# AssemblyAI-Community/MinImagen

Measured on NVIDIA H100. Metric: denoising steps/sec (SR256 U-Net, batch 32 per GPU per step), higher is better.
Workload: dtype f16 tensor-core operands, f32 accumulate / residual stream

## Files before the change

### minimagen_b200/csrc/conv_tc.cu

```cuda
#include "conv_tc.cuh"

#include <cuda_runtime.h>
#include <mutex>
#include <stdio.h>

#include "kernels.cuh"
#include "launch.cuh"
#include "ptx.cuh"
#include "sat_half.cuh"
#include "wgmma.cuh"

namespace mi {

namespace {

constexpr int kNumThreads = 384;
constexpr uint32_t kABytes = kConvBlockM * kConvBlockK * 2;
constexpr uint32_t kRingBudget = 192 * 1024;
constexpr uint32_t kAuxBytes = 512;
constexpr uint32_t kSmemMax = 227 * 1024;
constexpr int kProducerRegs = 40;
constexpr int kConsumerRegs = 232;
static_assert(128 * kProducerRegs + 256 * kConsumerRegs <= 65536, "register file overcommitted");
constexpr int kTurnBar = 2;
constexpr int kStatBar = 4;
constexpr uint32_t stat_scratch_bytes(int block_n) { return 2 * 4 * (block_n / 16 > 0 ? block_n / 16 : 1) * 2 * 8; }

template <int BLOCK_N>
struct Cfg {
    static constexpr uint32_t kBBytes = BLOCK_N * kConvBlockK * 2;
    static constexpr uint32_t kStageBytes = kABytes + kBBytes;
    static constexpr int kStages = (kRingBudget / kStageBytes) > 8 ? 8 : (kRingBudget / kStageBytes);
    static constexpr uint32_t kSmemBytes = kStages * kStageBytes + 1024  + kAuxBytes;
};

__device__ __forceinline__ float silu(float v) { return __fdividef(v, 1.0f + __expf(-v)); }

template <int BLOCK_N, bool GN, bool TR = false>
__global__ void __launch_bounds__(kNumThreads, 1)
conv_wg_kernel(const __grid_constant__ CUtensorMap tmA, const __grid_constant__ CUtensorMap tmA2,
               const __grid_constant__ CUtensorMap tmB, const __grid_constant__ CUtensorMap tmX,
               const __grid_constant__ CUtensorMap tmX2, const __grid_constant__ ConvTcArgs args,
               const __grid_constant__ GnPrologueArgs gn) {
    using C = Cfg<BLOCK_N>;
    constexpr int STAGES = C::kStages;
    static_assert(2 * STAGES * 8 <= 256, "barrier block overlaps the GroupNorm scratch");
    static_assert(!TR || (BLOCK_N == 256 && !GN), "the transposed tile is the cooperative 256-wide one");
    constexpr bool PP = !GN && !TR && BLOCK_N <= 128;
    constexpr int HALVES = PP ? 2 : 1;
    constexpr int TILE_PIX = TR ? BLOCK_N : kConvBlockM;

    extern __shared__ uint8_t smem_raw[];
    uint8_t* smem = reinterpret_cast<uint8_t*>((reinterpret_cast<uintptr_t>(smem_raw) + 1023) & ~uintptr_t(1023));
    uint64_t* bars = reinterpret_cast<uint64_t*>(smem + STAGES * C::kStageBytes);
    uint64_t* full_bar = bars;
    uint64_t* empty_bar = bars + STAGES;

    const int warp = threadIdx.x >> 5;
    const int lane = threadIdx.x & 31;
    const int wg = threadIdx.x >> 7;
    int* err = args.err_flag;

    if (threadIdx.x == 0) {
        ptx::prefetch_tensormap(&tmB);
        if (!GN) {
            ptx::prefetch_tensormap(&tmA);
            ptx::prefetch_tensormap(&tmA2);
        }
        for (int i = 0; i < STAGES; ++i) {
            ptx::mbar_init(&full_bar[i], GN ? 5 : 1);
            ptx::mbar_init(&empty_bar[i], PP ? 1 : 2);
        }
        ptx::fence_barrier_init();
    }
    __syncthreads();
    pdl_wait();

    const int num_tap_kb = args.num_taps * args.chunks_per_tap;
    const int num_kb = num_tap_kb + args.x_chunks;
    const int tiles_m = args.tiles_w * args.tiles_h * args.tiles_b;
    const int total_tiles = tiles_m * args.tiles_n;
    const int BW = 1 << args.bw_log2, BH = 1 << args.bh_log2;
    const int BB = TILE_PIX >> (args.bw_log2 + args.bh_log2);

    if (wg == 0) {
        if constexpr (!GN) {
            ptx::setmaxnreg_dec<kProducerRegs>();
            if (warp == 0) {
                int stage = 0;
                uint32_t phase = 0;
                for (int tile = blockIdx.x; tile < total_tiles; tile += gridDim.x) {
                    const int nt = tile % args.tiles_n;
                    const int mt = tile / args.tiles_n;
                    const int w0 = (mt % args.tiles_w) * BW;
                    const int h0 = ((mt / args.tiles_w) % args.tiles_h) * BH;
                    const int b0 = (mt / (args.tiles_w * args.tiles_h)) * BB;
                    const int n0 = nt * BLOCK_N;
                    for (int kb = 0; kb < num_kb; ++kb) {
                        ptx::mbar_wait(&empty_bar[stage], phase ^ 1, err, 100 + stage);
                        if (ptx::elect_one()) {
                            uint8_t* sa = smem + stage * C::kStageBytes + (TR ? kABytes : 0);
                            uint8_t* sb = smem + stage * C::kStageBytes + (TR ? 0 : kABytes);
                            ptx::mbar_arrive_expect_tx(&full_bar[stage], C::kStageBytes);
                            if (kb < num_tap_kb) {
                                const int t = kb / args.chunks_per_tap, j = kb - t * args.chunks_per_tap;
                                const int cw = w0 * args.in_stride + args.dw[t], ch = h0 * args.in_stride + args.dh[t];
                                if (j < args.a_split)
                                    ptx::tma_load_5d(&tmA, &full_bar[stage], sa, args.a_chan_off + j * kConvBlockK, cw, ch,
                                                     args.ph[t], b0);
                                else
                                    ptx::tma_load_5d(&tmA2, &full_bar[stage], sa,
                                                     args.a_chan_off2 + (j - args.a_split) * kConvBlockK, cw, ch, args.ph[t], b0);
                            } else {
                                const int jx = kb - num_tap_kb;
                                if (jx < args.x_split)
                                    ptx::tma_load_5d(&tmX, &full_bar[stage], sa, args.x_chan_off + jx * kConvBlockK, w0, h0, 0, b0);
                                else
                                    ptx::tma_load_5d(&tmX2, &full_bar[stage], sa,
                                                     args.x_chan_off2 + (jx - args.x_split) * kConvBlockK, w0, h0, 0, b0);
                            }
                            ptx::tma_load_2d(&tmB, &full_bar[stage], sb, kb * kConvBlockK, n0);
                        }
                        if (++stage == STAGES) { stage = 0; phase ^= 1; }
                    }
                }
                pdl_trigger();
            }
        } else {
            float* s_mean = reinterpret_cast<float*>(reinterpret_cast<uint8_t*>(bars) + 256);
            float* s_rstd = s_mean + 32;
            float* sA = reinterpret_cast<float*>(reinterpret_cast<uint8_t*>(bars) + kAuxBytes);
            const int tt = threadIdx.x;
            const int lq = tt & 7;
            const int prow = tt >> 3;
            const int C0 = gn.C0, C1 = gn.C1, Ctot = C0 + C1, Cg = Ctot / gn.groups;
            const int H = args.H, W = args.W;
            float* sB = sA + Ctot;
            int stage = 0;
            uint32_t phase = 0;
            int cur_b = -1;
            for (int tile = blockIdx.x; tile < total_tiles; tile += gridDim.x) {
                const int nt = tile % args.tiles_n;
                const int mt = tile / args.tiles_n;
                const int w0 = (mt % args.tiles_w) * BW;
                const int h0 = ((mt / args.tiles_w) % args.tiles_h) * BH;
                const int b = mt / (args.tiles_w * args.tiles_h);
                const int n0 = nt * BLOCK_N;
                if (b != cur_b) {
                    ptx::bar_sync(1, 128);
                    if (tt < gn.groups) {
                        const int g = tt;
                        double su = 0.0, sq = 0.0;
                        const int lo = g * Cg, hi = lo + Cg;
                        const int lo0 = min(lo, C0), hi0 = min(hi, C0);
                        for (int e = lo0 / 16; e < hi0 / 16; ++e) {
                            su += gn.stats0[((long long)b * (C0 / 16) + e) * 2];
                            sq += gn.stats0[((long long)b * (C0 / 16) + e) * 2 + 1];
                        }
                        const int lo1 = max(lo, C0) - C0, hi1 = max(hi, C0) - C0;
                        for (int e = lo1 / 16; e < hi1 / 16; ++e) {
                            su += (double)gn.scale1 * gn.stats1[((long long)b * (C1 / 16) + e) * 2];
                            sq += (double)gn.scale1 * (double)gn.scale1 * gn.stats1[((long long)b * (C1 / 16) + e) * 2 + 1];
                        }
                        const double n = (double)Cg * H * W;
                        const double mean = su / n;
                        double var = sq / n - mean * mean;
                        if (var < 0) var = 0;
                        s_mean[g] = (float)mean;
                        s_rstd[g] = (float)(1.0 / sqrt(var + (double)gn.eps));
                    }
                    ptx::bar_sync(1, 128);
                    for (int cc = tt; cc < Ctot; cc += 128) {
                        const int g = cc / Cg;
                        float a = s_rstd[g] * gn.gamma[cc];
                        float bb = gn.beta[cc] - s_mean[g] * a;
                        if (gn.scale_shift) {
                            const float sc = gn.scale_shift[(long long)b * gn.ss_ld + cc] + 1.0f;
                            const float shv = gn.scale_shift[(long long)b * gn.ss_ld + Ctot + cc];
                            a *= sc;
                            bb = bb * sc + shv;
                        }
                        if (cc >= C0) a *= gn.scale1;
                        sA[cc] = a;
                        sB[cc] = bb;
                    }
                    cur_b = b;
                    ptx::bar_sync(1, 128);
                }
                const long long img = (long long)b * H * W;
                for (int kb = 0; kb < num_kb; ++kb) {
                    const int t = kb / args.chunks_per_tap, j = kb - t * args.chunks_per_tap;
                    const int dh = args.dh[t], dw = args.dw[t];
                    const float* cA = sA + j * kConvBlockK + lq * 8;
                    const float* cB = sB + j * kConvBlockK + lq * 8;
                    const float4 a0 = *reinterpret_cast<const float4*>(cA), a1 = *reinterpret_cast<const float4*>(cA + 4);
                    const float4 b0 = *reinterpret_cast<const float4*>(cB), b1 = *reinterpret_cast<const float4*>(cB + 4);
                    const bool first = j < args.a_split;
                    const int Cs = first ? C0 : C1;
                    const float* src = (first ? gn.src0 + (long long)j * kConvBlockK
                                              : gn.src1 + (long long)(j - args.a_split) * kConvBlockK) + img * Cs + lq * 8;

                    ptx::mbar_wait(&empty_bar[stage], phase ^ 1, err, 600 + stage);
                    uint8_t* sa = smem + stage * C::kStageBytes;
                    if (warp == 0 && ptx::elect_one()) {
                        ptx::mbar_arrive_expect_tx(&full_bar[stage], C::kBBytes);
                        ptx::tma_load_2d(&tmB, &full_bar[stage], sa + kABytes, kb * kConvBlockK, n0);
                    }
                    float4 x0[8], x1[8];
                    bool ok[8];
#pragma unroll
                    for (int i = 0; i < 8; ++i) {
                        const int m = i * 16 + prow;
                        const int gw = w0 + (m & (BW - 1)) + dw;
                        const int gh = h0 + ((m >> args.bw_log2) & (BH - 1)) + dh;
                        ok[i] = gh >= 0 && gh < H && gw >= 0 && gw < W;
                        if (ok[i]) {
                            const float4* s4 = reinterpret_cast<const float4*>(src + ((long long)gh * W + gw) * Cs);
                            x0[i] = __ldg(s4);
                            x1[i] = __ldg(s4 + 1);
                        }
                    }
#pragma unroll
                    for (int i = 0; i < 8; ++i) {
                        const int m = i * 16 + prow;
                        uint4 o = make_uint4(0u, 0u, 0u, 0u);
                        if (ok[i]) {
                            const __half2 h0_ = sat_half2(silu(fmaf(x0[i].x, a0.x, b0.x)), silu(fmaf(x0[i].y, a0.y, b0.y)));
                            const __half2 h1_ = sat_half2(silu(fmaf(x0[i].z, a0.z, b0.z)), silu(fmaf(x0[i].w, a0.w, b0.w)));
                            const __half2 h2_ = sat_half2(silu(fmaf(x1[i].x, a1.x, b1.x)), silu(fmaf(x1[i].y, a1.y, b1.y)));
                            const __half2 h3_ = sat_half2(silu(fmaf(x1[i].z, a1.z, b1.z)), silu(fmaf(x1[i].w, a1.w, b1.w)));
                            o.x = *reinterpret_cast<const uint32_t*>(&h0_); o.y = *reinterpret_cast<const uint32_t*>(&h1_);
                            o.z = *reinterpret_cast<const uint32_t*>(&h2_); o.w = *reinterpret_cast<const uint32_t*>(&h3_);
                        }
                        *reinterpret_cast<uint4*>(sa + m * 128 + ((lq ^ (m & 7)) << 4)) = o;
                    }
                    ptx::fence_proxy_async_smem();
                    __syncwarp();
                    if (lane == 0) ptx::mbar_arrive(&full_bar[stage]);
                    if (++stage == STAGES) { stage = 0; phase ^= 1; }
                }
            }
            pdl_trigger();
        }
    } else {
        if constexpr (!GN) ptx::setmaxnreg_inc<kConsumerRegs>();
        const int cw = wg - 1;
        const int wq = warp & 3;
        const int cq = 2 * (lane & 3);
        float acc[HALVES][BLOCK_N / 2];
        int stage = 0;
        uint32_t phase = 0;
        auto skip = [&](int n) {
            stage += n % STAGES;
            phase ^= (uint32_t)(n / STAGES) & 1u;
            if (stage >= STAGES) { stage -= STAGES; phase ^= 1; }
        };
        if (PP) skip(cw * num_kb);
        int bw_r[2 * HALVES], bh_r[2 * HALVES], bb_r[2 * HALVES], bb_warp[HALVES];
#pragma unroll
        for (int h = 0; h < HALVES; ++h) {
            const int m_warp = (PP ? h : cw) * 64 + wq * 16;
            bb_warp[h] = m_warp >> (args.bw_log2 + args.bh_log2);
#pragma unroll
            for (int r = 0; r < 2; ++r) {
                const int m = m_warp + (lane >> 2) + 8 * r;
                bw_r[2 * h + r] = m & (BW - 1);
                bh_r[2 * h + r] = (m >> args.bw_log2) & (BH - 1);
                bb_r[2 * h + r] = m >> (args.bw_log2 + args.bh_log2);
            }
        }
        constexpr int NQ = BLOCK_N / 16 > 0 ? BLOCK_N / 16 : 1;
        const bool tile_stats = PP && args.stats != nullptr && BB == 1;
        double* st_red = reinterpret_cast<double*>(reinterpret_cast<uint8_t*>(bars) + kAuxBytes);
        const bool vec = args.out_sc == 1 && ((reinterpret_cast<uintptr_t>(args.out_f32) & 7) == 0) &&
                         ((reinterpret_cast<uintptr_t>(args.residual) & 7) == 0) &&
                         ((reinterpret_cast<uintptr_t>(args.out_f16) & 3) == 0);

        for (int tile = blockIdx.x + (PP ? cw : 0) * gridDim.x; tile < total_tiles; tile += (PP ? 2 : 1) * gridDim.x) {
            const int nt = tile % args.tiles_n;
            const int mt = tile / args.tiles_n;
            const int n0 = nt * BLOCK_N;
            if (PP && tile != (int)blockIdx.x) ptx::bar_sync(kTurnBar + cw, 256);
            int prev = -1;
            for (int kb = 0; kb < num_kb; ++kb) {
                ptx::mbar_wait(&full_bar[stage], phase, err, 300 + stage);
                const uint32_t sa = ptx::smem_u32(smem + stage * C::kStageBytes);
                const uint64_t db = ptx::make_sw128_desc(sa + kABytes);
                ptx::wg_fence();
#pragma unroll
                for (int k = 0; k < kConvBlockK / 16; ++k)
#pragma unroll
                    for (int h = 0; h < HALVES; ++h) {
                        const uint64_t da = ptx::make_sw128_desc(sa + (PP ? h : cw) * (64 * 128));
                        ptx::Wgmma<BLOCK_N, 0>::run(acc[h], da + 2 * k, db + 2 * k, (kb | k) != 0);
                    }
                ptx::wg_commit();
                ptx::wg_wait<1>();
                if (prev >= 0 && (threadIdx.x & 127) == 0) ptx::mbar_arrive(&empty_bar[prev]);
                prev = stage;
                if (++stage == STAGES) { stage = 0; phase ^= 1; }
            }
            if (PP && tile + (int)gridDim.x < total_tiles) ptx::bar_arrive(kTurnBar + (cw ^ 1), 256);
            if (PP) skip(num_kb);
            ptx::wg_wait<0>();
#pragma unroll
            for (int h = 0; h < HALVES; ++h) ptx::wg_fence_regs(acc[h]);
            if (prev >= 0 && (threadIdx.x & 127) == 0) ptx::mbar_arrive(&empty_bar[prev]);

            const int tw0 = (mt % args.tiles_w) * BW;
            const int th0 = ((mt / args.tiles_w) % args.tiles_h) * BH;
            const int tb0 = (mt / (args.tiles_w * args.tiles_h)) * BB;
            if constexpr (TR) {
                const int c0 = 64 * cw + 16 * wq + (lane >> 2);
                const float bv[2] = {args.bias ? __ldg(args.bias + c0) : 0.f, args.bias ? __ldg(args.bias + c0 + 8) : 0.f};
                const long long base = (long long)tb0 * args.out_sb + (long long)th0 * args.out_sh +
                                       (long long)(tw0 + cq) * args.out_sw + c0;
                float* const o32 = args.out_f32 ? args.out_f32 + base : nullptr;
                __half* const o16 = args.out_f16 ? args.out_f16 + base : nullptr;
                const float* const res = args.residual ? args.residual + base : nullptr;
                const int sw = (int)args.out_sw, step = 8 * sw, wrap = (int)args.out_sh - (BW - 8) * sw;
                float* a = acc[0];
                int oj = 0;
#pragma unroll
                for (int j = 0; j < BLOCK_N / 8; ++j) {
                    if (j > 0) oj += ((8 * j) & (BW - 1)) ? step : wrap;
#pragma unroll
                    for (int r = 0; r < 2; ++r)
#pragma unroll
                        for (int e = 0; e < 2; ++e) {
                            float& f = a[4 * j + 2 * r + e];
                            f += bv[r];
                            if (res) f += res[oj + e * sw + 8 * r];
                        }
                }
                const bool stats = args.stats != nullptr;
                double su = 0.0, sq = 0.0;
                oj = 0;
#pragma unroll
                for (int jj = 0; jj < BLOCK_N / 16; ++jj) {
                    float s8 = 0.f, q8 = 0.f;
#pragma unroll
                    for (int j = 2 * jj; j < 2 * jj + 2; ++j) {
                        if (j > 0) oj += ((8 * j) & (BW - 1)) ? step : wrap;
#pragma unroll
                        for (int r = 0; r < 2; ++r) {
                            const float* f = a + 4 * j + 2 * r;
#pragma unroll
                            for (int e = 0; e < 2; ++e) {
                                const int o = oj + e * sw + 8 * r;
                                if (o32) o32[o] = f[e];
                                if (o16) o16[o] = sat_half(f[e]);
                            }
                            if (stats) {
                                s8 += f[0] + f[1];
                                q8 += f[0] * f[0] + f[1] * f[1];
                            }
                        }
                    }
                    if (stats) {
                        su += (double)s8;
// ... 177 lines not shown
        if (tiles_m * (Cout / cands[i]) >= num_sms || cands[i] <= 64) break;
    }
    return block_n;
}

CUresult encode_act(PFN_encodeTiled enc, CUtensorMap* m, const void* ptr, cuuint64_t channels, cuuint64_t ld, int W, int H,
                    int phases, int B, int in_stride, int tile_pix, const ConvTcArgs& a) {
    const cuuint64_t IS = in_stride;
    const int BW = 1 << a.bw_log2, BH = 1 << a.bh_log2, BB = tile_pix >> (a.bw_log2 + a.bh_log2);
    cuuint64_t gdim[5] = {channels, (cuuint64_t)W * IS, (cuuint64_t)H * IS, (cuuint64_t)phases, (cuuint64_t)B};
    cuuint64_t gstr[4] = {ld * 2, (cuuint64_t)W * IS * ld * 2, (cuuint64_t)H * IS * W * IS * ld * 2,
                          (cuuint64_t)phases * H * IS * W * IS * ld * 2};
    cuuint32_t box[5] = {kConvBlockK, (cuuint32_t)(BW * IS), (cuuint32_t)(BH * IS), 1, (cuuint32_t)BB};
    cuuint32_t estr[5] = {1, (cuuint32_t)IS, (cuuint32_t)IS, 1, 1};
    return enc(m, CU_TENSOR_MAP_DATA_TYPE_FLOAT16, 5, const_cast<void*>(ptr), gdim, gstr, box, estr,
               CU_TENSOR_MAP_INTERLEAVE_NONE, CU_TENSOR_MAP_SWIZZLE_128B, CU_TENSOR_MAP_L2_PROMOTION_L2_256B,
               CU_TENSOR_MAP_FLOAT_OOB_FILL_NONE);
}

CUresult encode_weights(PFN_encodeTiled enc, CUtensorMap* m, const void* ptr, cuuint64_t K, int Cout, int block_n) {
    cuuint64_t gdim[2] = {K, (cuuint64_t)Cout};
    cuuint64_t gstr[1] = {K * 2};
    cuuint32_t box[2] = {kConvBlockK, (cuuint32_t)block_n};
    cuuint32_t estr[2] = {1, 1};
    return enc(m, CU_TENSOR_MAP_DATA_TYPE_FLOAT16, 2, const_cast<void*>(ptr), gdim, gstr, box, estr,
               CU_TENSOR_MAP_INTERLEAVE_NONE, CU_TENSOR_MAP_SWIZZLE_128B, CU_TENSOR_MAP_L2_PROMOTION_L2_256B,
               CU_TENSOR_MAP_FLOAT_OOB_FILL_NONE);
}

bool transposed_ok(const ConvTcProblem& p, const ConvTcArgs& a) {
    if (p.Cout != 128 || a.n_valid != p.Cout || a.out_sc != 1) return false;
    int BW, BH;
    tile_box(p.H, p.W, 256, BW, BH);
    if (p.W % BW || ilog2_exact(BW) < 3 || BW * a.in_stride > 256 || BW * BH != 256) return false;
    if (BH * a.out_sh + BW * a.out_sw + p.Cout > INT32_MAX) return false;
    return p.H % BH == 0 && BH * a.in_stride <= 256;
}

template <int BLOCK_N, bool GN, bool TR = false>
int launch(const CUtensorMap& tmA, const CUtensorMap& tmA2, const CUtensorMap& tmB, const CUtensorMap& tmX,
           const CUtensorMap& tmX2, const ConvTcArgs& args, const GnPrologueArgs& gn, uint32_t extra_smem,
           cudaStream_t stream) {
    using C = Cfg<BLOCK_N>;
    static bool attr_set = false;
    if (!attr_set) {
        if (cudaFuncSetAttribute(conv_wg_kernel<BLOCK_N, GN, TR>, cudaFuncAttributeMaxDynamicSharedMemorySize, kSmemMax) !=
            cudaSuccess)
            return -10;
        attr_set = true;
    }
    const int total_tiles = args.tiles_w * args.tiles_h * args.tiles_b * args.tiles_n;
    const int num_sms = num_sms_of_current_device();
    const int grid = total_tiles < num_sms ? total_tiles : num_sms;
    const uint32_t smem = C::kSmemBytes + (!GN && !TR && BLOCK_N <= 128 ? stat_scratch_bytes(BLOCK_N) : 0u) + extra_smem;
    launch_k(conv_wg_kernel<BLOCK_N, GN, TR>, grid, kNumThreads, smem, stream, tmA, tmA2, tmB, tmX, tmX2, args, gn);
    return cudaGetLastError() == cudaSuccess ? 0 : -11;
}

}

PFN_tmaEncodeTiled get_tma_encode() { return get_encode(); }

const char* conv_tc_strerror(int code) {
    switch (code) {
        case 0: return "ok";
        case -1: return "conv_tc: C_in (per tap) must be a positive multiple of 64";
        case -2: return "conv_tc: C_out must be a multiple of 16";
        case -3: return "conv_tc: W must be >= 128, a power of two >= 8, or a multiple of 8 whose largest power-of-two divisor BW gives " \
                       "128 / BW rows dividing H";
        case -4: return "conv_tc: too many taps (max 16)";
        case -5: return "conv_tc: cuTensorMapEncodeTiled unavailable";
        case -6: return "conv_tc: tensor map encode failed (activations)";
        case -7: return "conv_tc: tensor map encode failed (weights)";
        case -8: return "conv_tc: pointer/stride alignment (16 B) violated";
        case -9: return "conv_tc: the folded 1x1 operand needs a stride-1 conv over one phase";
        case -10: return "conv_tc: cudaFuncSetAttribute(max dynamic smem) failed";
        case -11: return "conv_tc: kernel launch failed";
        default: return "conv_tc: unknown error";
    }
}

bool conv_tc_supported(int H, int W, int Cin, int Cout) {
    if (Cin <= 0 || Cin % kConvBlockK != 0 || Cout <= 0 || Cout % 16 != 0) return false;
    if (W >= 128) return true;
    if (ilog2_exact(W) < 0) {
        const int low = W & -W;
        return W > 0 && low >= 8 && H % (128 / low) == 0;
    }
    if (W < 8) return false;
    const int bh = 128 / W;
    if (H >= bh) return H % bh == 0;
    return ilog2_exact(H) >= 0;
}

int conv_tc_launch(const ConvTcProblem& p, cudaStream_t stream) {
    if (p.Cin <= 0 || p.Cin % kConvBlockK != 0) return -1;
    if (p.Cout % 16 != 0) return -2;
    if (p.num_taps < 1 || p.num_taps > kConvMaxTaps) return -4;
    if (!conv_tc_supported(p.H, p.W, p.Cin, p.Cout)) return -3;
    if ((reinterpret_cast<uintptr_t>(p.act) & 15) || (reinterpret_cast<uintptr_t>(p.wpacked) & 15) ||
        (p.lda % 8) != 0)
        return -8;
    PFN_encodeTiled enc = get_encode();
    if (!enc) return -5;

    ConvTcArgs a{};
    a.num_taps = p.num_taps;
// ... 15 lines not shown
                                : (hint == 0 || p.Cout % hint != 0) && tr_ok && (long long)p.B * p.H * p.W / 256 >= num_sms;
    const int tile_pix = tr ? 256 : kConvBlockM;
    tile_geometry(p.H, p.W, p.B, tile_pix, a);
    const int tiles_m = a.tiles_w * a.tiles_h * a.tiles_b;
    const int block_n = tr ? 128 : pick_block_n(p.Cout, tiles_m, p.block_n_hint, num_sms);
    a.tiles_n = p.Cout / block_n;

    CUtensorMap tmA, tmA2, tmB, tmX, tmX2;
    a.a_split = (p.act2 ? p.Cin1 : p.Cin) / kConvBlockK;
    a.a_chan_off2 = p.a_chan_off2;
    if (encode_act(enc, &tmA, p.act, p.a_channels, p.lda, p.W, p.H, p.phases, p.B, a.in_stride, tile_pix, a) != CUDA_SUCCESS)
        return -6;
    tmA2 = tmA;
    if (p.act2) {
        if (p.Cin1 <= 0 || p.Cin1 % kConvBlockK || p.Cin1 >= p.Cin || (p.lda2 % 8) || (reinterpret_cast<uintptr_t>(p.act2) & 15) ||
            a.in_stride != 1)
            return -8;
        if (encode_act(enc, &tmA2, p.act2, p.lda2, p.lda2, p.W, p.H, p.phases, p.B, 1, tile_pix, a) != CUDA_SUCCESS) return -6;
    }
    tmX = tmA; tmX2 = tmA;
    if (p.x_act) {
        if (p.phases != 1 || a.in_stride != 1) return -9;
        if (p.Cx <= 0 || p.Cx % kConvBlockK || (p.x_lda % 8) || (reinterpret_cast<uintptr_t>(p.x_act) & 15)) return -8;
        if (p.x_act2 && (p.Cx1 <= 0 || p.Cx1 % kConvBlockK || p.Cx1 >= p.Cx || (p.x_lda2 % 8) ||
                         (reinterpret_cast<uintptr_t>(p.x_act2) & 15)))
            return -8;
        a.x_chunks = p.Cx / kConvBlockK;
        a.x_split = (p.x_act2 ? p.Cx1 : p.Cx) / kConvBlockK;
        a.x_chan_off = p.x_chan_off; a.x_chan_off2 = p.x_chan_off2;
        if (encode_act(enc, &tmX, p.x_act, p.x_lda, p.x_lda, p.W, p.H, 1, p.B, 1, tile_pix, a) != CUDA_SUCCESS) return -6;
        tmX2 = tmX;
        if (p.x_act2 &&
            encode_act(enc, &tmX2, p.x_act2, p.x_lda2, p.x_lda2, p.W, p.H, 1, p.B, 1, tile_pix, a) != CUDA_SUCCESS)
            return -6;
    }
    const cuuint64_t K = (cuuint64_t)p.num_taps * p.Cin + (p.x_act ? (cuuint64_t)p.Cx : 0);
    if (encode_weights(enc, &tmB, p.wpacked, K, p.Cout, block_n) != CUDA_SUCCESS) return -7;

    const GnPrologueArgs gn{};
    if (tr) return launch<256, false, true>(tmA, tmA2, tmB, tmX, tmX2, a, gn, 0, stream);
    switch (block_n) {
        case 256: return launch<256, false>(tmA, tmA2, tmB, tmX, tmX2, a, gn, 0, stream);
        case 128: return launch<128, false>(tmA, tmA2, tmB, tmX, tmX2, a, gn, 0, stream);
        case 64: return launch<64, false>(tmA, tmA2, tmB, tmX, tmX2, a, gn, 0, stream);
        case 32: return launch<32, false>(tmA, tmA2, tmB, tmX, tmX2, a, gn, 0, stream);
        default: return launch<16, false>(tmA, tmA2, tmB, tmX, tmX2, a, gn, 0, stream);
    }
}


bool conv_gn_supported(int H, int W, int C0, int C1, int Cout, int groups) {
    const int C = C0 + C1;
    if (H <= 0 || W <= 0 || H % 32 || W % 8 || C0 <= 0 || C0 % 64 || C1 < 0 || C1 % 64 || Cout <= 0 || Cout % 128) return false;
    if (!conv_tc_supported(H, W, C, Cout) || H * W < kConvBlockM) return false;
    if (groups < 1 || groups > 32 || C % groups) return false;
    if (Cfg<128>::kSmemBytes + 8u * (uint32_t)C > kSmemMax) return false;
    return (C / groups) % 16 == 0;
}

int conv_gn_launch(const ConvGnProblem& p, cudaStream_t stream) {
    if (!conv_gn_supported(p.H, p.W, p.C0, p.C1, p.Cout, p.groups)) return -3;
    if (p.C1 && (!p.src1 || !p.stats1)) return -8;
    if (!p.src0 || !p.stats0 || !p.gamma || !p.beta) return -8;
    if ((reinterpret_cast<uintptr_t>(p.src0) & 15) || (reinterpret_cast<uintptr_t>(p.src1) & 15) ||
        (reinterpret_cast<uintptr_t>(p.wpacked) & 15))
        return -8;
    PFN_encodeTiled enc = get_encode();
    if (!enc) return -5;
    const int C = p.C0 + p.C1;

    ConvTcArgs a{};
    a.num_taps = 9;
    for (int t = 0; t < 9; ++t) { a.dh[t] = (int8_t)(t / 3 - 1); a.dw[t] = (int8_t)(t % 3 - 1); a.ph[t] = 0; }
    a.chunks_per_tap = C / kConvBlockK;
    a.a_split = p.C0 / kConvBlockK;
    a.in_stride = 1;
    tile_geometry(p.H, p.W, p.B, kConvBlockM, a);
    a.out_sb = (long long)p.H * p.W * p.Cout; a.out_sh = (long long)p.W * p.Cout; a.out_sw = p.Cout; a.out_sc = 1;
    a.n_valid = p.Cout;
    a.out_f32 = p.out_f32; a.out_f16 = p.out_f16; a.bias = p.bias; a.residual = p.residual; a.err_flag = p.err_flag;
    a.stats = p.out_stats; a.stats_blocks = p.Cout / 16;
    a.tiles_n = p.Cout / 128;

    GnPrologueArgs g{};
    g.src0 = p.src0; g.src1 = p.src1;
    g.C0 = p.C0; g.C1 = p.C1; g.groups = p.groups; g.scale1 = p.scale1; g.eps = p.eps;
    g.stats0 = p.stats0; g.stats1 = p.stats1; g.gamma = p.gamma; g.beta = p.beta;
    g.scale_shift = p.scale_shift; g.ss_ld = p.ss_ld;

    CUtensorMap tmB;
    if (encode_weights(enc, &tmB, p.wpacked, (cuuint64_t)9 * C, p.Cout, 128) != CUDA_SUCCESS) return -7;
    return launch<128, true>(tmB, tmB, tmB, tmB, tmB, a, g, 8u * (uint32_t)C, stream);
}

}
```

### minimagen_b200/csrc/ptx.cuh

```cuda
#pragma once
#include <cuda.h>
#include <cuda_fp16.h>
#include <stdint.h>

namespace mi {
namespace ptx {

__device__ __forceinline__ uint32_t smem_u32(const void* p) {
    return static_cast<uint32_t>(__cvta_generic_to_shared(p));
}

__device__ __forceinline__ void mbar_init(uint64_t* bar, uint32_t count) {
    asm volatile("mbarrier.init.shared::cta.b64 [%0], %1;" ::"r"(smem_u32(bar)), "r"(count));
}
__device__ __forceinline__ void fence_barrier_init() {
    asm volatile("fence.mbarrier_init.release.cluster;" ::: "memory");
}
__device__ __forceinline__ void fence_proxy_async_smem() {
    asm volatile("fence.proxy.async.shared::cta;" ::: "memory");
}
__device__ __forceinline__ void mbar_arrive(uint64_t* bar) {
    asm volatile("mbarrier.arrive.shared::cta.b64 _, [%0];" ::"r"(smem_u32(bar)) : "memory");
}
__device__ __forceinline__ void mbar_arrive_expect_tx(uint64_t* bar, uint32_t bytes) {
// ... 1 lines not shown
                 : "memory");
}
__device__ __forceinline__ bool mbar_try_wait(uint64_t* bar, uint32_t parity) {
    uint32_t ok;
    asm volatile(
        "{\n\t"
        ".reg .pred p;\n\t"
        "mbarrier.try_wait.parity.shared::cta.b64 p, [%1], %2;\n\t"
        "selp.u32 %0, 1, 0, p;\n\t"
        "}"
        : "=r"(ok)
        : "r"(smem_u32(bar)), "r"(parity)
        : "memory");
    return ok != 0;
}
__device__ __forceinline__ void mbar_wait(uint64_t* bar, uint32_t parity, int* err, int code) {
    if (mbar_try_wait(bar, parity)) return;
    const long long t0 = clock64();
    while (!mbar_try_wait(bar, parity)) {
        if (clock64() - t0 > 4000000000LL) {
            if (err) { atomicExch(err, code); __threadfence_system(); }
            __trap();
        }
    }
}

__device__ __forceinline__ bool elect_one() {
    uint32_t pred;
    asm volatile("{\n .reg .pred p;\n elect.sync _|p, 0xffffffff;\n selp.u32 %0, 1, 0, p;\n}" : "=r"(pred));
    return pred != 0;
}

__device__ __forceinline__ float ex2_approx(float x) {
    float y;
    asm("ex2.approx.ftz.f32 %0, %1;" : "=f"(y) : "f"(x));
    return y;
}

__device__ __forceinline__ int ld_acquire_gpu(const int* p) {
    int v;
    asm volatile("ld.acquire.gpu.global.s32 %0, [%1];" : "=r"(v) : "l"(p) : "memory");
    return v;
}

__device__ __forceinline__ void prefetch_tensormap(const CUtensorMap* m) {
    asm volatile("prefetch.tensormap [%0];" ::"l"(reinterpret_cast<uint64_t>(m)) : "memory");
}
__device__ __forceinline__ void tma_load_2d(const CUtensorMap* m, uint64_t* bar, void* dst, int c0, int c1) {
    asm volatile(
        "cp.async.bulk.tensor.2d.shared::cluster.global.mbarrier::complete_tx::bytes [%0], [%1, {%3, %4}], [%2];"
        ::"r"(smem_u32(dst)), "l"(reinterpret_cast<uint64_t>(m)), "r"(smem_u32(bar)), "r"(c0), "r"(c1)
        : "memory");
}
__device__ __forceinline__ void tma_load_5d(const CUtensorMap* m, uint64_t* bar, void* dst, int c0, int c1, int c2,
                                            int c3, int c4) {
    asm volatile(
        "cp.async.bulk.tensor.5d.shared::cluster.global.mbarrier::complete_tx::bytes [%0], [%1, {%3, %4, %5, %6, "
        "%7}], [%2];"
        ::"r"(smem_u32(dst)), "l"(reinterpret_cast<uint64_t>(m)), "r"(smem_u32(bar)), "r"(c0), "r"(c1), "r"(c2),
        "r"(c3), "r"(c4)
        : "memory");
}

__device__ __forceinline__ void wg_fence() { asm volatile("wgmma.fence.sync.aligned;" ::: "memory"); }
__device__ __forceinline__ void wg_commit() { asm volatile("wgmma.commit_group.sync.aligned;" ::: "memory"); }
template <int N>
__device__ __forceinline__ void wg_wait() { asm volatile("wgmma.wait_group.sync.aligned %0;" ::"n"(N) : "memory"); }
template <int R>
__device__ __forceinline__ void wg_fence_regs(float (&d)[R]) {
#pragma unroll
    for (int i = 0; i < R; ++i) asm volatile("" : "+f"(d[i])::"memory");
}

__device__ __forceinline__ uint64_t make_sw128_desc(uint32_t smem_addr, uint32_t lbo_bytes = 16) {
    uint64_t d = 0;
    d |= static_cast<uint64_t>((smem_addr >> 4) & 0x3FFF);
    d |= static_cast<uint64_t>((lbo_bytes >> 4) & 0x3FFF) << 16;
    d |= static_cast<uint64_t>(1024u >> 4) << 32;
    d |= static_cast<uint64_t>(1) << 62;
    return d;
}
__device__ __forceinline__ void bar_sync(int id, int count) {
    asm volatile("bar.sync %0, %1;" ::"r"(id), "r"(count) : "memory");
}
__device__ __forceinline__ void bar_arrive(int id, int count) {
    asm volatile("bar.arrive %0, %1;" ::"r"(id), "r"(count) : "memory");
}

template <int N>
__device__ __forceinline__ void setmaxnreg_dec() { asm volatile("setmaxnreg.dec.sync.aligned.u32 %0;" ::"n"(N)); }
template <int N>
__device__ __forceinline__ void setmaxnreg_inc() { asm volatile("setmaxnreg.inc.sync.aligned.u32 %0;" ::"n"(N)); }

}
}
```

Before: 16.64.

## Stage GroupNorm conv input as normalized halo tile reused across all nine taps

The fused GroupNorm+SiLU conv path now loads each 64-channel chunk once per tile as an fp32 halo box (8x16 pixels plus a one-pixel border) via TMA. It normalizes it into a double-buffered f16 halo in shared memory and feeds all nine taps from that halo using non-swizzled wgmma descriptors. Before, each tap re-read the input from global memory and re-applied the normalization. A dedicated warp now streams only weights through a deeper ring, registers are rebalanced between producer and consumer groups, and 256-wide output tiles are used when Cout allows. The cost is a much more complex barrier scheme, a fixed tile geometry, and non-swizzled smem operands that may cause bank conflicts.

```diff
diff --git a/minimagen_b200/csrc/conv_tc.cu b/minimagen_b200/csrc/conv_tc.cu
--- a/minimagen_b200/csrc/conv_tc.cu
+++ b/minimagen_b200/csrc/conv_tc.cu
@@ -22,6 +22,9 @@
 constexpr int kProducerRegs = 40;
 constexpr int kConsumerRegs = 232;
 static_assert(128 * kProducerRegs + 256 * kConsumerRegs <= 65536, "register file overcommitted");
+constexpr int kGnProducerRegs = 72;
+constexpr int kGnConsumerRegs = 216;
+static_assert(128 * kGnProducerRegs + 256 * kGnConsumerRegs <= kNumThreads * 168, "register split exceeds the launch's registers");
 constexpr int kTurnBar = 2;
 constexpr int kStatBar = 4;
 constexpr uint32_t stat_scratch_bytes(int block_n) { return 2 * 4 * (block_n / 16 > 0 ? block_n / 16 : 1) * 2 * 8; }
@@ -34,6 +37,23 @@
     static constexpr uint32_t kSmemBytes = kStages * kStageBytes + 1024  + kAuxBytes;
 };
 
+constexpr int kHaloW = 10, kHaloH = 18, kHaloPix = kHaloW * kHaloH;
+constexpr uint32_t kHaloGroupBytes = kHaloPix * 16 + 16;
+constexpr uint32_t kHaloSlot = (8 * kHaloGroupBytes + 1023) / 1024 * 1024;
+constexpr uint32_t kStgBytes = kHaloPix * kConvBlockK * 4;
+constexpr int kGnMaxC = 2048;
+template <int BLOCK_N>
+struct GnCfg {
+    static constexpr uint32_t kBBytes = BLOCK_N * kConvBlockK * 2;
+    static constexpr uint32_t kFixed = 2 * kHaloSlot + kStgBytes + 1024  + kAuxBytes;
+    static constexpr int kStages0 = (kSmemMax - kFixed - 8 * kGnMaxC) / kBBytes;
+    static constexpr int kStages = kStages0 > 8 ? 8 : kStages0;
+    static constexpr uint32_t kHaloOff = kStages * kBBytes, kStgOff = kHaloOff + 2 * kHaloSlot, kBarOff = kStgOff + kStgBytes;
+    static constexpr uint32_t kSmemBytes = kBarOff + 1024 + kAuxBytes;
+    static_assert(kStages >= 3, "fewer than three weight stages");
+    static_assert(kSmemBytes + 8 * kGnMaxC <= kSmemMax, "shared memory budget of the fused GroupNorm conv");
+};
+
 __device__ __forceinline__ float silu(float v) { return __fdividef(v, 1.0f + __expf(-v)); }
 
 template <int BLOCK_N, bool GN, bool TR = false>
@@ -43,8 +63,10 @@
                const __grid_constant__ CUtensorMap tmX2, const __grid_constant__ ConvTcArgs args,
                const __grid_constant__ GnPrologueArgs gn) {
     using C = Cfg<BLOCK_N>;
-    constexpr int STAGES = C::kStages;
-    static_assert(2 * STAGES * 8 <= 256, "barrier block overlaps the GroupNorm scratch");
+    using G = GnCfg<BLOCK_N>;
+    constexpr int STAGES = GN ? G::kStages : C::kStages;
+    constexpr uint32_t SLOT = GN ? G::kBBytes : C::kStageBytes;
+    static_assert((2 * STAGES + 5) * 8 <= 256, "barrier block overlaps the GroupNorm scratch");
     static_assert(!TR || (BLOCK_N == 256 && !GN), "the transposed tile is the cooperative 256-wide one");
     constexpr bool PP = !GN && !TR && BLOCK_N <= 128;
     constexpr int HALVES = PP ? 2 : 1;
@@ -52,9 +74,12 @@
 
     extern __shared__ uint8_t smem_raw[];
     uint8_t* smem = reinterpret_cast<uint8_t*>((reinterpret_cast<uintptr_t>(smem_raw) + 1023) & ~uintptr_t(1023));
-    uint64_t* bars = reinterpret_cast<uint64_t*>(smem + STAGES * C::kStageBytes);
+    uint64_t* bars = reinterpret_cast<uint64_t*>(smem + (GN ? G::kBarOff : STAGES * C::kStageBytes));
     uint64_t* full_bar = bars;
     uint64_t* empty_bar = bars + STAGES;
+    uint64_t* halo_full = bars + 2 * STAGES;
+    uint64_t* halo_empty = halo_full + 2;
+    uint64_t* stg_full = halo_full + 4;
 
     const int warp = threadIdx.x >> 5;
     const int lane = threadIdx.x & 31;
@@ -63,13 +88,18 @@
 
     if (threadIdx.x == 0) {
         ptx::prefetch_tensormap(&tmB);
-        if (!GN) {
-            ptx::prefetch_tensormap(&tmA);
-            ptx::prefetch_tensormap(&tmA2);
+        ptx::prefetch_tensormap(&tmA);
+        ptx::prefetch_tensormap(&tmA2);
+        for (int i = 0; i < STAGES; ++i) {
+            ptx::mbar_init(&full_bar[i], 1);
+            ptx::mbar_init(&empty_bar[i], PP ? 1 : 2);
         }
-        for (int i = 0; i < STAGES; ++i) {
-            ptx::mbar_init(&full_bar[i], GN ? 5 : 1);
-            ptx::mbar_init(&empty_bar[i], PP ? 1 : 2);
+        if (GN) {
+            for (int i = 0; i < 2; ++i) {
+                ptx::mbar_init(&halo_full[i], 3);
+                ptx::mbar_init(&halo_empty[i], 2);
+            }
+            ptx::mbar_init(stg_full, 1);
         }
         ptx::fence_barrier_init();
     }
@@ -84,8 +114,8 @@
     const int BB = TILE_PIX >> (args.bw_log2 + args.bh_log2);
 
     if (wg == 0) {
+        ptx::setmaxnreg_dec<GN ? kGnProducerRegs : kProducerRegs>();
         if constexpr (!GN) {
-            ptx::setmaxnreg_dec<kProducerRegs>();
             if (warp == 0) {
                 int stage = 0;
                 uint32_t phase = 0;
@@ -127,129 +157,143 @@
                 pdl_trigger();
             }
         } else {
-            float* s_mean = reinterpret_cast<float*>(reinterpret_cast<uint8_t*>(bars) + 256);
-            float* s_rstd = s_mean + 32;
-            float* sA = reinterpret_cast<float*>(reinterpret_cast<uint8_t*>(bars) + kAuxBytes);
-            const int tt = threadIdx.x;
-            const int lq = tt & 7;
-            const int prow = tt >> 3;
-            const int C0 = gn.C0, C1 = gn.C1, Ctot = C0 + C1, Cg = Ctot / gn.groups;
+            const int C0 = gn.C0, C1 = gn.C1, Ctot = C0 + C1, Cc = args.chunks_per_tap;
             const int H = args.H, W = args.W;
-            float* sB = sA + Ctot;
-            int stage = 0;
-            uint32_t phase = 0;
-            int cur_b = -1;
-            for (int tile = blockIdx.x; tile < total_tiles; tile += gridDim.x) {
-                const int nt = tile % args.tiles_n;
-                const int mt = tile / args.tiles_n;
-                const int w0 = (mt % args.tiles_w) * BW;
-                const int h0 = ((mt / args.tiles_w) % args.tiles_h) * BH;
-                const int b = mt / (args.tiles_w * args.tiles_h);
-                const int n0 = nt * BLOCK_N;
-                if (b != cur_b) {
-                    ptx::bar_sync(1, 128);
-                    if (tt < gn.groups) {
-                        const int g = tt;
-                        double su = 0.0, sq = 0.0;
-                        const int lo = g * Cg, hi = lo + Cg;
-                        const int lo0 = min(lo, C0), hi0 = min(hi, C0);
-                        for (int e = lo0 / 16; e < hi0 / 16; ++e) {
-                            su += gn.stats0[((long long)b * (C0 / 16) + e) * 2];
-                            sq += gn.stats0[((long long)b * (C0 / 16) + e) * 2 + 1];
-                        }
-                        const int lo1 = max(lo, C0) - C0, hi1 = max(hi, C0) - C0;
-                        for (int e = lo1 / 16; e < hi1 / 16; ++e) {
-                            su += (double)gn.scale1 * gn.stats1[((long long)b * (C1 / 16) + e) * 2];
-                            sq += (double)gn.scale1 * (double)gn.scale1 * gn.stats1[((long long)b * (C1 / 16) + e) * 2 + 1];
-                        }
-                        const double n = (double)Cg * H * W;
-                        const double mean = su / n;
-                        double var = sq / n - mean * mean;
-                        if (var < 0) var = 0;
-                        s_mean[g] = (float)mean;
-                        s_rstd[g] = (float)(1.0 / sqrt(var + (double)gn.eps));
-                    }
-                    ptx::bar_sync(1, 128);
-                    for (int cc = tt; cc < Ctot; cc += 128) {
-                        const int g = cc / Cg;
-                        float a = s_rstd[g] * gn.gamma[cc];
-                        float bb = gn.beta[cc] - s_mean[g] * a;
-                        if (gn.scale_shift) {
-                            const float sc = gn.scale_shift[(long long)b * gn.ss_ld + cc] + 1.0f;
-                            const float shv = gn.scale_shift[(long long)b * gn.ss_ld + Ctot + cc];
-                            a *= sc;
-                            bb = bb * sc + shv;
-                        }
-                        if (cc >= C0) a *= gn.scale1;
-                        sA[cc] = a;
-                        sB[cc] = bb;
-                    }
-                    cur_b = b;
-                    ptx::bar_sync(1, 128);
-                }
-                const long long img = (long long)b * H * W;
-                for (int kb = 0; kb < num_kb; ++kb) {
-                    const int t = kb / args.chunks_per_tap, j = kb - t * args.chunks_per_tap;
-                    const int dh = args.dh[t], dw = args.dw[t];
-                    const float* cA = sA + j * kConvBlockK + lq * 8;
-                    const float* cB = sB + j * kConvBlockK + lq * 8;
-                    const float4 a0 = *reinterpret_cast<const float4*>(cA), a1 = *reinterpret_cast<const float4*>(cA + 4);
-                    const float4 b0 = *reinterpret_cast<const float4*>(cB), b1 = *reinterpret_cast<const float4*>(cB + 4);
-                    const bool first = j < args.a_split;
-                    const int Cs = first ? C0 : C1;
-                    const float* src = (first ? gn.src0 + (long long)j * kConvBlockK
-                                              : gn.src1 + (long long)(j - args.a_split) * kConvBlockK) + img * Cs + lq * 8;
-
-                    ptx::mbar_wait(&empty_bar[stage], phase ^ 1, err, 600 + stage);
-                    uint8_t* sa = smem + stage * C::kStageBytes;
-                    if (warp == 0 && ptx::elect_one()) {
-                        ptx::mbar_arrive_expect_tx(&full_bar[stage], C::kBBytes);
-                        ptx::tma_load_2d(&tmB, &full_bar[stage], sa + kABytes, kb * kConvBlockK, n0);
-                    }
-                    float4 x0[8], x1[8];
-                    bool ok[8];
-#pragma unroll
-                    for (int i = 0; i < 8; ++i) {
-                        const int m = i * 16 + prow;
-                        const int gw = w0 + (m & (BW - 1)) + dw;
-                        const int gh = h0 + ((m >> args.bw_log2) & (BH - 1)) + dh;
-                        ok[i] = gh >= 0 && gh < H && gw >= 0 && gw < W;
-                        if (ok[i]) {
-                            const float4* s4 = reinterpret_cast<const float4*>(src + ((long long)gh * W + gw) * Cs);
-                            x0[i] = __ldg(s4);
-                            x1[i] = __ldg(s4 + 1);
-                        }
-                    }
-#pragma unroll
-                    for (int i = 0; i < 8; ++i) {
-                        const int m = i * 16 + prow;
-                        uint4 o = make_uint4(0u, 0u, 0u, 0u);
-                        if (ok[i]) {
-                            const __half2 h0_ = sat_half2(silu(fmaf(x0[i].x, a0.x, b0.x)), silu(fmaf(x0[i].y, a0.y, b0.y)));
-                            const __half2 h1_ = sat_half2(silu(fmaf(x0[i].z, a0.z, b0.z)), silu(fmaf(x0[i].w, a0.w, b0.w)));
-                            const __half2 h2_ = sat_half2(silu(fmaf(x1[i].x, a1.x, b1.x)), silu(fmaf(x1[i].y, a1.y, b1.y)));
-                            const __half2 h3_ = sat_half2(silu(fmaf(x1[i].z, a1.z, b1.z)), silu(fmaf(x1[i].w, a1.w, b1.w)));
-                            o.x = *reinterpret_cast<const uint32_t*>(&h0_); o.y = *reinterpret_cast<const uint32_t*>(&h1_);
-                            o.z = *reinterpret_cast<const uint32_t*>(&h2_); o.w = *reinterpret_cast<const uint32_t*>(&h3_);
-                        }
-                        *reinterpret_cast<uint4*>(sa + m * 128 + ((lq ^ (m & 7)) << 4)) = o;
-                    }
-                    ptx::fence_proxy_async_smem();
-                    __syncwarp();
-                    if (lane == 0) ptx::mbar_arrive(&full_bar[stage]);
-                    if (++stage == STAGES) { stage = 0; phase ^= 1; }
+            if (warp == 0) {
+                int stage = 0;
+                uint32_t phase = 0;
+                for (int tile = blockIdx.x; tile < total_tiles; tile += gridDim.x) {
+                    const int n0 = (tile % args.tiles_n) * BLOCK_N;
+                    for (int j = 0; j < Cc; ++j)
+                        for (int t = 0; t < 9; ++t) {
+                            ptx::mbar_wait(&empty_bar[stage], phase ^ 1, err, 100 + stage);
+                            if (ptx::elect_one()) {
+                                ptx::mbar_arrive_expect_tx(&full_bar[stage], G::kBBytes);
+                                ptx::tma_load_2d(&tmB, &full_bar[stage], smem + stage * SLOT, t * Ctot + j * kConvBlockK, n0);
+                            }
+                            if (++stage == STAGES) { stage = 0; phase ^= 1; }
+                        }
+                }
+            } else {
+                float* s_mean = reinterpret_cast<float*>(reinterpret_cast<uint8_t*>(bars) + 256);
+                float* s_rstd = s_mean + 32;
+                float* sA = reinterpret_cast<float*>(reinterpret_cast<uint8_t*>(bars) + kAuxBytes);
+                float* sB = sA + Ctot;
+                const float* stg = reinterpret_cast<const float*>(smem + G::kStgOff);
+                const int tq = threadIdx.x - 32;
+                const int Cg = Ctot / gn.groups;
+                auto load_box = [&](int tile, int j) {
+                    if (tile >= total_tiles) return;
+                    const int mt = tile / args.tiles_n;
+                    const int w0 = (mt % args.tiles_w) * BW, h0 = ((mt / args.tiles_w) % args.tiles_h) * BH;
+                    const int b = mt / (args.tiles_w * args.tiles_h);
+                    ptx::mbar_arrive_expect_tx(stg_full, kStgBytes);
+                    if (j < args.a_split)
+                        ptx::tma_load_4d(&tmA, stg_full, smem + G::kStgOff, j * kConvBlockK, w0 - 1, h0 - 1, b);
+                    else
+                        ptx::tma_load_4d(&tmA2, stg_full, smem + G::kStgOff, (j - args.a_split) * kConvBlockK, w0 - 1, h0 - 1, b);
+                };
+                if (warp == 1 && ptx::elect_one()) load_box(blockIdx.x, 0);
+                int hs = 0;
+                uint32_t hphase = 0, sphase = 0;
+                int cur_b = -1;
+                for (int tile = blockIdx.x; tile < total_tiles; tile += gridDim.x) {
+                    const int mt = tile / args.tiles_n;
+                    const int w0 = (mt % args.tiles_w) * BW;
+                    const int h0 = ((mt / args.tiles_w) % args.tiles_h) * BH;
+                    const int b = mt / (args.tiles_w * args.tiles_h);
+                    if (b != cur_b) {
+                        if (tq < gn.groups) {
+                            const int g = tq;
+                            double su = 0.0, sq = 0.0;
+                            const int lo = g * Cg, hi = lo + Cg;
+                            const int lo0 = min(lo, C0), hi0 = min(hi, C0);
+                            for (int e = lo0 / 16; e < hi0 / 16; ++e) {
+                                su += gn.stats0[((long long)b * (C0 / 16) + e) * 2];
+                                sq += gn.stats0[((long long)b * (C0 / 16) + e) * 2 + 1];
+                            }
+                            const int lo1 = max(lo, C0) - C0, hi1 = max(hi, C0) - C0;
+                            for (int e = lo1 / 16; e < hi1 / 16; ++e) {
+                                su += (double)gn.scale1 * gn.stats1[((long long)b * (C1 / 16) + e) * 2];
+                                sq += (double)gn.scale1 * (double)gn.scale1 * gn.stats1[((long long)b * (C1 / 16) + e) * 2 + 1];
+                            }
+                            const double n = (double)Cg * H * W;
+                            const double mean = su / n;
+                            double var = sq / n - mean * mean;
+                            if (var < 0) var = 0;
+                            s_mean[g] = (float)mean;
+                            s_rstd[g] = (float)(1.0 / sqrt(var + (double)gn.eps));
+                        }
+                        ptx::bar_sync(1, 96);
+                        for (int cc = tq; cc < Ctot; cc += 96) {
+                            const int g = cc / Cg;
+                            float a = s_rstd[g] * gn.gamma[cc];
+                            float bb = gn.beta[cc] - s_mean[g] * a;
+                            if (gn.scale_shift) {
+                                const float sc = gn.scale_shift[(long long)b * gn.ss_ld + cc] + 1.0f;
+                                const float shv = gn.scale_shift[(long long)b * gn.ss_ld + Ctot + cc];
+                                a *= sc;
+                                bb = bb * sc + shv;
+                            }
+                            if (cc >= C0) a *= gn.scale1;
+                            sA[cc] = a;
+                            sB[cc] = bb;
+                        }
+                        cur_b = b;
+                        ptx::bar_sync(1, 96);
+                    }
+                    for (int j = 0; j < Cc; ++j) {
+                        uint8_t* halo = smem + G::kHaloOff + hs * kHaloSlot;
+                        ptx::mbar_wait(&halo_empty[hs], hphase ^ 1, err, 600 + hs);
+                        const int q = tq & 7;
+                        const float* cA = sA + j * kConvBlockK + q * 8;
+                        const float* cB = sB + j * kConvBlockK + q * 8;
+                        const float4 a0 = *reinterpret_cast<const float4*>(cA), a1 = *reinterpret_cast<const float4*>(cA + 4);
+                        const float4 b0 = *reinterpret_cast<const float4*>(cB), b1 = *reinterpret_cast<const float4*>(cB + 4);
+                        ptx::mbar_wait(stg_full, sphase, err, 610);
+                        sphase ^= 1;
+#pragma unroll 3
+                        for (int p = tq >> 3; p < kHaloPix; p += 12) {
+                            const int hh = p / kHaloW, ww = p - hh * kHaloW;
+                            const int gh = h0 - 1 + hh, gw = w0 - 1 + ww;
+                            uint4 o = make_uint4(0u, 0u, 0u, 0u);
+                            if (gh >= 0 && gh < H && gw >= 0 && gw < W) {
+                                const float4 x0 = *reinterpret_cast<const float4*>(stg + p * kConvBlockK + q * 8);
+                                const float4 x1 = *reinterpret_cast<const float4*>(stg + p * kConvBlockK + q * 8 + 4);
+                                const __half2 h0_ = sat_half2(silu(fmaf(x0.x, a0.x, b0.x)), silu(fmaf(x0.y, a0.y, b0.y)));
+                                const __half2 h1_ = sat_half2(silu(fmaf(x0.z, a0.z, b0.z)), silu(fmaf(x0.w, a0.w, b0.w)));
+                                const __half2 h2_ = sat_half2(silu(fmaf(x1.x, a1.x, b1.x)), silu(fmaf(x1.y, a1.y, b1.y)));
+                                const __half2 h3_ = sat_half2(silu(fmaf(x1.z, a1.z, b1.z)), silu(fmaf(x1.w, a1.w, b1.w)));
+                                o.x = *reinterpret_cast<const uint32_t*>(&h0_); o.y = *reinterpret_cast<const uint32_t*>(&h1_);
+                                o.z = *reinterpret_cast<const uint32_t*>(&h2_); o.w = *reinterpret_cast<const uint32_t*>(&h3_);
+                            }
+                            *reinterpret_cast<uint4*>(halo + q * kHaloGroupBytes + p * 16) = o;
+                        }
+                        ptx::fence_proxy_async_smem();
+                        __syncwarp();
+                        if (lane == 0) ptx::mbar_arrive(&halo_full[hs]);
+                        ptx::bar_sync(1, 96);
+                        if (warp == 1 && ptx::elect_one()) {
+                            ptx::fence_proxy_async_smem();
+                            if (j + 1 < Cc) load_box(tile, j + 1);
+                            else load_box(tile + gridDim.x, 0);
+                        }
+                        if (++hs == 2) { hs = 0; hphase ^= 1; }
+                    }
                 }
             }
             pdl_trigger();
         }
     } else {
-        if constexpr (!GN) ptx::setmaxnreg_inc<kConsumerRegs>();
+        ptx::setmaxnreg_inc<GN ? kGnConsumerRegs : kConsumerRegs>();
         const int cw = wg - 1;
         const int wq = warp & 3;
         const int cq = 2 * (lane & 3);
         float acc[HALVES][BLOCK_N / 2];
         int stage = 0;
         uint32_t phase = 0;
+        int hs = 0;
+        uint32_t hphase = 0;
         auto skip = [&](int n) {
             stage += n % STAGES;
             phase ^= (uint32_t)(n / STAGES) & 1u;
@@ -282,30 +326,66 @@
             const int n0 = nt * BLOCK_N;
             if (PP && tile != (int)blockIdx.x) ptx::bar_sync(kTurnBar + cw, 256);
             int prev = -1;
-            for (int kb = 0; kb < num_kb; ++kb) {
-                ptx::mbar_wait(&full_bar[stage], phase, err, 300 + stage);
-                const uint32_t sa = ptx::smem_u32(smem + stage * C::kStageBytes);
-                const uint64_t db = ptx::make_sw128_desc(sa + kABytes);
-                ptx::wg_fence();
-#pragma unroll
-                for (int k = 0; k < kConvBlockK / 16; ++k)
-#pragma unroll
-                    for (int h = 0; h < HALVES; ++h) {
-                        const uint64_t da = ptx::make_sw128_desc(sa + (PP ? h : cw) * (64 * 128));
-                        ptx::Wgmma<BLOCK_N, 0>::run(acc[h], da + 2 * k, db + 2 * k, (kb | k) != 0);
-                    }
-                ptx::wg_commit();
-                ptx::wg_wait<1>();
+            if constexpr (GN) {
+                int prev_h = -1;
+                for (int j = 0; j < args.chunks_per_tap; ++j) {
+                    ptx::mbar_wait(&halo_full[hs], hphase, err, 700 + hs);
+                    const uint32_t hb = ptx::smem_u32(smem + G::kHaloOff + hs * kHaloSlot);
+#pragma unroll 1
+                    for (int t = 0; t < 9; ++t) {
+                        ptx::mbar_wait(&full_bar[stage], phase, err, 300 + stage);
+                        const uint64_t db = ptx::make_sw128_desc(ptx::smem_u32(smem + stage * SLOT));
+                        const uint64_t da = ptx::make_nosw_desc(
+                            hb + (uint32_t)(((8 * cw + t / 3) * kHaloW + t % 3) * 16), kHaloGroupBytes, kHaloW * 16);
+                        ptx::wg_fence();
+#pragma unroll
+                        for (int k = 0; k < kConvBlockK / 16; ++k)
+                            ptx::Wgmma<BLOCK_N, 0>::run(acc[0], da + k * (2 * kHaloGroupBytes >> 4), db + 2 * k,
+                                                        (j | t | k) != 0);
+                        ptx::wg_commit();
+                        ptx::wg_wait<1>();
+                        if ((threadIdx.x & 127) == 0) {
+                            if (prev >= 0) ptx::mbar_arrive(&empty_bar[prev]);
+                            if (t == 0 && prev_h >= 0) ptx::mbar_arrive(&halo_empty[prev_h]);
+                        }
+                        prev = stage;
+                        if (++stage == STAGES) { stage = 0; phase ^= 1; }
+                    }
+                    prev_h = hs;
+                    if (++hs == 2) { hs = 0; hphase ^= 1; }
+                }
+                ptx::wg_wait<0>();
+                ptx::wg_fence_regs(acc[0]);
+                if ((threadIdx.x & 127) == 0) {
+                    ptx::mbar_arrive(&empty_bar[prev]);
+                    ptx::mbar_arrive(&halo_empty[prev_h]);
+                }
+            } else {
+                for (int kb = 0; kb < num_kb; ++kb) {
+                    ptx::mbar_wait(&full_bar[stage], phase, err, 300 + stage);
+                    const uint32_t sa = ptx::smem_u32(smem + stage * C::kStageBytes);
+                    const uint64_t db = ptx::make_sw128_desc(sa + kABytes);
+                    ptx::wg_fence();
+    #pragma unroll
+                    for (int k = 0; k < kConvBlockK / 16; ++k)
+    #pragma unroll
+                        for (int h = 0; h < HALVES; ++h) {
+                            const uint64_t da = ptx::make_sw128_desc(sa + (PP ? h : cw) * (64 * 128));
+                            ptx::Wgmma<BLOCK_N, 0>::run(acc[h], da + 2 * k, db + 2 * k, (kb | k) != 0);
+                        }
+                    ptx::wg_commit();
+                    ptx::wg_wait<1>();
+                    if (prev >= 0 && (threadIdx.x & 127) == 0) ptx::mbar_arrive(&empty_bar[prev]);
+                    prev = stage;
+                    if (++stage == STAGES) { stage = 0; phase ^= 1; }
+                }
+                if (PP && tile + (int)gridDim.x < total_tiles) ptx::bar_arrive(kTurnBar + (cw ^ 1), 256);
+                if (PP) skip(num_kb);
+                ptx::wg_wait<0>();
+    #pragma unroll
+                for (int h = 0; h < HALVES; ++h) ptx::wg_fence_regs(acc[h]);
                 if (prev >= 0 && (threadIdx.x & 127) == 0) ptx::mbar_arrive(&empty_bar[prev]);
-                prev = stage;
-                if (++stage == STAGES) { stage = 0; phase ^= 1; }
             }
-            if (PP && tile + (int)gridDim.x < total_tiles) ptx::bar_arrive(kTurnBar + (cw ^ 1), 256);
-            if (PP) skip(num_kb);
-            ptx::wg_wait<0>();
-#pragma unroll
-            for (int h = 0; h < HALVES; ++h) ptx::wg_fence_regs(acc[h]);
-            if (prev >= 0 && (threadIdx.x & 127) == 0) ptx::mbar_arrive(&empty_bar[prev]);
 
             const int tw0 = (mt % args.tiles_w) * BW;
             const int th0 = ((mt / args.tiles_w) % args.tiles_h) * BH;
@@ -589,7 +669,8 @@
     const int total_tiles = args.tiles_w * args.tiles_h * args.tiles_b * args.tiles_n;
     const int num_sms = num_sms_of_current_device();
     const int grid = total_tiles < num_sms ? total_tiles : num_sms;
-    const uint32_t smem = C::kSmemBytes + (!GN && !TR && BLOCK_N <= 128 ? stat_scratch_bytes(BLOCK_N) : 0u) + extra_smem;
+    const uint32_t smem = (GN ? GnCfg<BLOCK_N>::kSmemBytes : C::kSmemBytes) +
+                          (!GN && !TR && BLOCK_N <= 128 ? stat_scratch_bytes(BLOCK_N) : 0u) + extra_smem;
     launch_k(conv_wg_kernel<BLOCK_N, GN, TR>, grid, kNumThreads, smem, stream, tmA, tmA2, tmB, tmX, tmX2, args, gn);
     return cudaGetLastError() == cudaSuccess ? 0 : -11;
 }
@@ -711,10 +792,19 @@
 bool conv_gn_supported(int H, int W, int C0, int C1, int Cout, int groups) {
     const int C = C0 + C1;
     if (H <= 0 || W <= 0 || H % 32 || W % 8 || C0 <= 0 || C0 % 64 || C1 < 0 || C1 % 64 || Cout <= 0 || Cout % 128) return false;
-    if (!conv_tc_supported(H, W, C, Cout) || H * W < kConvBlockM) return false;
-    if (groups < 1 || groups > 32 || C % groups) return false;
-    if (Cfg<128>::kSmemBytes + 8u * (uint32_t)C > kSmemMax) return false;
+    if (!conv_tc_supported(H, W, C, Cout)) return false;
+    if (groups < 1 || groups > 32 || C % groups || C > kGnMaxC) return false;
     return (C / groups) % 16 == 0;
+}
+
+CUresult encode_halo_src(PFN_encodeTiled enc, CUtensorMap* m, const float* ptr, int C, int W, int H, int B) {
+    cuuint64_t gdim[4] = {(cuuint64_t)C, (cuuint64_t)W, (cuuint64_t)H, (cuuint64_t)B};
+    cuuint64_t gstr[3] = {(cuuint64_t)C * 4, (cuuint64_t)W * C * 4, (cuuint64_t)H * W * C * 4};
+    cuuint32_t box[4] = {kConvBlockK, kHaloW, kHaloH, 1};
+    cuuint32_t estr[4] = {1, 1, 1, 1};
+    return enc(m, CU_TENSOR_MAP_DATA_TYPE_FLOAT32, 4, const_cast<float*>(ptr), gdim, gstr, box, estr,
+               CU_TENSOR_MAP_INTERLEAVE_NONE, CU_TENSOR_MAP_SWIZZLE_NONE, CU_TENSOR_MAP_L2_PROMOTION_L2_256B,
+               CU_TENSOR_MAP_FLOAT_OOB_FILL_NONE);
 }
 
 int conv_gn_launch(const ConvGnProblem& p, cudaStream_t stream) {
@@ -734,12 +824,15 @@
     a.chunks_per_tap = C / kConvBlockK;
     a.a_split = p.C0 / kConvBlockK;
     a.in_stride = 1;
-    tile_geometry(p.H, p.W, p.B, kConvBlockM, a);
+    a.bw_log2 = 3; a.bh_log2 = 4;
+    a.tiles_w = p.W / 8; a.tiles_h = p.H / 16; a.tiles_b = p.B;
+    a.B = p.B; a.H = p.H; a.W = p.W;
     a.out_sb = (long long)p.H * p.W * p.Cout; a.out_sh = (long long)p.W * p.Cout; a.out_sw = p.Cout; a.out_sc = 1;
     a.n_valid = p.Cout;
     a.out_f32 = p.out_f32; a.out_f16 = p.out_f16; a.bias = p.bias; a.residual = p.residual; a.err_flag = p.err_flag;
     a.stats = p.out_stats; a.stats_blocks = p.Cout / 16;
-    a.tiles_n = p.Cout / 128;
+    const int block_n = p.Cout % 256 == 0 ? 256 : 128;
+    a.tiles_n = p.Cout / block_n;
 
     GnPrologueArgs g{};
     g.src0 = p.src0; g.src1 = p.src1;
@@ -747,9 +840,13 @@
     g.stats0 = p.stats0; g.stats1 = p.stats1; g.gamma = p.gamma; g.beta = p.beta;
     g.scale_shift = p.scale_shift; g.ss_ld = p.ss_ld;
 
-    CUtensorMap tmB;
-    if (encode_weights(enc, &tmB, p.wpacked, (cuuint64_t)9 * C, p.Cout, 128) != CUDA_SUCCESS) return -7;
-    return launch<128, true>(tmB, tmB, tmB, tmB, tmB, a, g, 8u * (uint32_t)C, stream);
-}
-
-}
+    CUtensorMap tmA, tmA2, tmB;
+    if (encode_halo_src(enc, &tmA, p.src0, p.C0, p.W, p.H, p.B) != CUDA_SUCCESS) return -6;
+    tmA2 = tmA;
+    if (p.C1 && encode_halo_src(enc, &tmA2, p.src1, p.C1, p.W, p.H, p.B) != CUDA_SUCCESS) return -6;
+    if (encode_weights(enc, &tmB, p.wpacked, (cuuint64_t)9 * C, p.Cout, block_n) != CUDA_SUCCESS) return -7;
+    if (block_n == 256) return launch<256, true>(tmA, tmA2, tmB, tmB, tmB, a, g, 8u * (uint32_t)C, stream);
+    return launch<128, true>(tmA, tmA2, tmB, tmB, tmB, a, g, 8u * (uint32_t)C, stream);
+}
+
+}
diff --git a/minimagen_b200/csrc/ptx.cuh b/minimagen_b200/csrc/ptx.cuh
--- a/minimagen_b200/csrc/ptx.cuh
+++ b/minimagen_b200/csrc/ptx.cuh
@@ -77,6 +77,13 @@
         ::"r"(smem_u32(dst)), "l"(reinterpret_cast<uint64_t>(m)), "r"(smem_u32(bar)), "r"(c0), "r"(c1)
         : "memory");
 }
+__device__ __forceinline__ void tma_load_4d(const CUtensorMap* m, uint64_t* bar, void* dst, int c0, int c1, int c2,
+                                            int c3) {
+    asm volatile(
+        "cp.async.bulk.tensor.4d.shared::cluster.global.mbarrier::complete_tx::bytes [%0], [%1, {%3, %4, %5, %6}], [%2];"
+        ::"r"(smem_u32(dst)), "l"(reinterpret_cast<uint64_t>(m)), "r"(smem_u32(bar)), "r"(c0), "r"(c1), "r"(c2), "r"(c3)
+        : "memory");
+}
 __device__ __forceinline__ void tma_load_5d(const CUtensorMap* m, uint64_t* bar, void* dst, int c0, int c1, int c2,
                                             int c3, int c4) {
     asm volatile(
@@ -105,6 +112,13 @@
     d |= static_cast<uint64_t>(1) << 62;
     return d;
 }
+__device__ __forceinline__ uint64_t make_nosw_desc(uint32_t smem_addr, uint32_t lbo_bytes, uint32_t sbo_bytes) {
+    uint64_t d = 0;
+    d |= static_cast<uint64_t>((smem_addr >> 4) & 0x3FFF);
+    d |= static_cast<uint64_t>((lbo_bytes >> 4) & 0x3FFF) << 16;
+    d |= static_cast<uint64_t>((sbo_bytes >> 4) & 0x3FFF) << 32;
+    return d;
+}
 __device__ __forceinline__ void bar_sync(int id, int count) {
     asm volatile("bar.sync %0, %1;" ::"r"(id), "r"(count) : "memory");
 }
```

Measured after the change: 16.67, median of 6. Within noise of the previous version (+0.2%).
